# RoadlyInc/DSOPP

Hardware: AMD Instinct MI355X
Metric: Gauss-Newton iters/sec (7-KF window, 2k active pts) (higher is better)
Workload: dtype f64; 1 GPU; C1: 7-KF window, 2000 active points per GPU (2000 total, 2000 on rank 0), 640x480, full clique, production LM settings; frames=7, points_per_gpu=2000, total_points=2000, parallelism=single GPU, exchange=none, ranks=1

## Files before the change

dsopp_amd/csrc/pba_kernels.hpp:

```cpp
#pragma once
#include <type_traits>
#include "device_geom.hpp"
#include "pba_types.hpp"

namespace dsopp_hip {

__device__ __constant__ const int kPatX[kPat] = {0, -1, 1, -2, 0, 2, -1, 0};
__device__ __constant__ const int kPatY[kPat] = {2, 1, 1, 0, 0, 0, -1, -2};

__host__ __device__ constexpr int triIdx(int i, int j) { return i * kBlk - i * (i - 1) / 2 + (j - i); }
__host__ __device__ inline int symIdx(int i, int j) { return i <= j ? triIdx(i, j) : triIdx(j, i); }

__device__ inline void buildProjectionMatrices(const Rigid &T, const FrameDev &fr, const FrameDev &ft, double *U, double *M) {
  const double ifx = 1.0 / fr.fx, ify = 1.0 / fr.fy;
  const double k02 = -fr.cx / fr.fx, k12 = -fr.cy / fr.fy;
#pragma unroll
  for (int i = 0; i < 3; ++i) {
    U[4 * i + 0] = T.R[3 * i + 0] * ifx;
    U[4 * i + 1] = T.R[3 * i + 1] * ify;
    U[4 * i + 2] = T.R[3 * i + 0] * k02 + T.R[3 * i + 1] * k12 + T.R[3 * i + 2];
    U[4 * i + 3] = T.t[i];
  }
  if (M) {
#pragma unroll
    for (int j = 0; j < 4; ++j) {
      M[0 + j] = ft.fx * U[0 + j] + ft.cx * U[8 + j];
      M[4 + j] = ft.fy * U[4 + j] + ft.cy * U[8 + j];
      M[8 + j] = U[8 + j];
    }
  }
}

template <typename FramesPtr, typename StatePtr>
__device__ __forceinline__ double linearisationScale(FramesPtr frames, StatePtr st, int r, int t) {
  return (frames[t].exposure / frames[r].exposure) * exp(st->ab0[t][0] - st->ab0[r][0]);
}

template <typename StatePtr>
__device__ __forceinline__ Rigid frameIncrement(StatePtr st, int f, double sign) {
  double xi[6];
#pragma unroll
  for (int i = 0; i < 6; ++i) xi[i] = sign * (st->eps[f][i] + st->step[f][i]);
  return rigidExp(xi);
}

template <int PART = 0>
__device__ __forceinline__ void computePairConst(const FrameDev *frames_generic, const WindowState *st_generic, PairConst *pc_generic, int r, int t,
                                                 int F, bool fej, const Rigid *Er = nullptr, const Rigid *Emt = nullptr) {
  const auto frames = glb(frames_generic);
  const auto st = glb(st_generic);
  auto &P = glb(pc_generic)[r * kMaxFrames + t];
  const auto &fr = frames[r];
  const auto &ft = frames[t];
  const bool valid = (r != t) && fr.status[t] != nullptr;
  if (PART != 2) P.valid = valid ? 1 : 0;
  if (!valid) return;
  Rigid Tr0, Tt0;
#pragma unroll
  for (int i = 0; i < 9; ++i) {
    Tr0.R[i] = st->T0_R[r][i];
    Tt0.R[i] = st->T0_R[t][i];
  }
#pragma unroll
  for (int i = 0; i < 3; ++i) {
    Tr0.t[i] = st->T0_t[r][i];
    Tt0.t[i] = st->T0_t[t][i];
  }
  const Rigid T_tr0 = rigidMul(rigidInverse(Tt0), Tr0);
  if (PART != 1) {
#pragma unroll
    for (int i = 0; i < 3; ++i) {
#pragma unroll
      for (int j = 0; j < 3; ++j) P.T0rel[4 * i + j] = T_tr0.R[3 * i + j];
      P.T0rel[4 * i + 3] = T_tr0.t[i];
    }
  }
  FrameDev ir{}, it{};
  ir.fx = fr.fx;
  ir.fy = fr.fy;
  ir.cx = fr.cx;
  ir.cy = fr.cy;
  it.fx = ft.fx;
  it.fy = ft.fy;
  it.cx = ft.cx;
  it.cy = ft.cy;
  const bool need_current = PART != 2 || !fej;
  Rigid T_tr = T_tr0;
  double b_r = 0, s_cur = 0;
  if (need_current) {
    T_tr = rigidMul(Emt ? *Emt : frameIncrement(st, t, -1.0), rigidMul(T_tr0, Er ? *Er : frameIncrement(st, r, 1.0)));
    const double a_r = st->ab0[r][0] + st->eps[r][6] + st->step[r][6];
    const double a_t = st->ab0[t][0] + st->eps[t][6] + st->step[t][6];
    b_r = st->ab0[r][1] + st->eps[r][7] + st->step[r][7];
    s_cur = (ft.exposure / fr.exposure) * exp(a_t - a_r);
  }
  if (PART != 2) {
    const double b_t = st->ab0[t][1] + st->eps[t][7] + st->step[t][7];
    P.s = s_cur;
    P.b_t = b_t;
    P.b_r = b_r;
    double Ucur[12], Mcur[12];
    buildProjectionMatrices(T_tr, ir, it, Ucur, Mcur);
#pragma unroll
    for (int i = 0; i < 12; ++i) P.M[i] = Mcur[i];
  }
  if (PART != 1) {
    const Rigid Tlin = fej ? T_tr0 : T_tr;
    double Ulin[12], adj[36];
    buildProjectionMatrices(Tlin, ir, it, Ulin, nullptr);
    rigidAdj(Tlin, adj);
#pragma unroll
    for (int i = 0; i < 12; ++i) P.U[i] = Ulin[i];
#pragma unroll
    for (int i = 0; i < 36; ++i) P.Adj[i] = adj[i];
#pragma unroll
    for (int i = 0; i < 3; ++i) P.tl[i] = Tlin.t[i];
    P.fxt = ft.fx;
    P.fyt = ft.fy;
    P.cxt = ft.cx;
    P.cyt = ft.cy;
    if (fej) {
      P.s0 = linearisationScale(frames, st, r, t);
      P.b_r0 = st->ab0[r][1];
      int last = -1;
      for (int k = 0; k < F; ++k)
        if (k != r && fr.status[k] != nullptr) last = k;
      P.sigma_r = linearisationScale(frames, st, r, last);
    } else {
      P.s0 = s_cur;
      P.b_r0 = b_r;
      P.sigma_r = s_cur;
    }
  }
}

__device__ inline void refreshPairCurrent(const FrameDev *frames, const WindowState *st, PairConst *pc, int r, int t, const Rigid &Er,
                                          const Rigid &Emt) {
  PairConst &P = pc[r * kMaxFrames + t];
  if (!P.valid) return;
  Rigid T0;
#pragma unroll
  for (int i = 0; i < 3; ++i) {
#pragma unroll
    for (int j = 0; j < 3; ++j) T0.R[3 * i + j] = P.T0rel[4 * i + j];
    T0.t[i] = P.T0rel[4 * i + 3];
  }
  const Rigid T_tr = rigidMul(Emt, rigidMul(T0, Er));
  const FrameDev &fr = frames[r];
  const FrameDev &ft = frames[t];
  double U[12];
  buildProjectionMatrices(T_tr, fr, ft, U, P.M);
  const double a_r = st->ab0[r][0] + st->eps[r][6] + st->step[r][6];
  const double a_t = st->ab0[t][0] + st->eps[t][6] + st->step[t][6];
  P.s = (ft.exposure / fr.exposure) * exp(a_t - a_r);
  P.b_t = st->ab0[t][1] + st->eps[t][7] + st->step[t][7];
  P.b_r = st->ab0[r][1] + st->eps[r][7] + st->step[r][7];
}

__global__ void __launch_bounds__(kMaxFrames *kMaxFrames) pairSetupKernel(const FrameDev *frames, const WindowState *st, PairConst *pc, int F, int fej,
                                                                          const int *run_flag) {
  if (run_flag && !*run_flag) return;
  const int idx = threadIdx.x;
  if (idx >= F * F) return;
  computePairConst(frames, st, pc, idx / F, idx % F, F, fej != 0);
}

__device__ __forceinline__ double waveSum(double v) {
#pragma unroll
  for (int off = 32; off >= 1; off >>= 1) v += __shfl_xor(v, off, 64);
  return v;
}

__device__ __forceinline__ double waveSumDpp(double v) {
  auto mov = [](double x, auto ctrl_tag) {
    constexpr int CTRL = decltype(ctrl_tag)::value;
    int lo = __double2loint(x), hi = __double2hiint(x);
    lo = __builtin_amdgcn_mov_dpp(lo, CTRL, 0xF, 0xF, true);
    hi = __builtin_amdgcn_mov_dpp(hi, CTRL, 0xF, 0xF, true);
    return __hiloint2double(hi, lo);
  };
  v += mov(v, std::integral_constant<int, 0xB1>{});
  v += mov(v, std::integral_constant<int, 0x4E>{});
  v += mov(v, std::integral_constant<int, 0x141>{});
  v += mov(v, std::integral_constant<int, 0x140>{});
  auto row = [&](int lane) {
    const int lo = __builtin_amdgcn_readlane(__double2loint(v), lane), hi = __builtin_amdgcn_readlane(__double2hiint(v), lane);
    return __hiloint2double(hi, lo);
  };
  return ((row(0) + row(16)) + row(32)) + row(48);
}

template <int N, int THREADS>
__device__ __forceinline__ void blockSum(double (&vals)[N], double *lds ) {
  constexpr int kWaves = THREADS / 64;
  const int lane = threadIdx.x & 63, wave = threadIdx.x >> 6;
#pragma unroll
  for (int i = 0; i < N; ++i) vals[i] = waveSum(vals[i]);
  if (kWaves > 1) {
    if (lane == 0) {
#pragma unroll
      for (int i = 0; i < N; ++i) lds[wave * N + i] = vals[i];
    }
    __syncthreads();
    if (threadIdx.x == 0) {
#pragma unroll
      for (int i = 0; i < N; ++i) {
        double s = lds[i];
        for (int w = 1; w < kWaves; ++w) s += lds[w * N + i];
        vals[i] = s;
      }
    }
  }
}

constexpr int kItemsPerBlock = kSweepThreads / kPat;

template <typename S>
__global__ void __launch_bounds__(64) fejKernel(const FrameDev *__restrict__ frames, const PairConst *__restrict__ pc,
                                                const SweepBlock *__restrict__ table, int n_entries) {
  const int entry = blockIdx.x * (64 / kItemsPerBlock) + (threadIdx.x / kItemsPerBlock);
  if (entry >= n_entries) return;
  const SweepBlock be = table[entry];
  const FrameDev &fr = frames[be.r];
  const FrameDev &ft = frames[be.t];
  const PairConst &P = pc[be.r * kMaxFrames + be.t];
  const int i = be.offset + threadIdx.x % kItemsPerBlock;
  if (i >= fr.n_res[be.t]) return;
  const uint8_t flg = fr.flags[i];
  if ((flg & kFlagMarginalized) && !(flg & kFlagToMarginalize)) return;
  const S u = static_cast<S>(fr.uv[2 * i]), v = static_cast<S>(fr.uv[2 * i + 1]);
  const double idepth_d = fr.idepth[i];
  const S idepth = static_cast<S>(idepth_d);
  bool ok = validIdepth(idepth) && insideROI(u - S(2), v - S(2), S(fr.width), S(fr.height)) &&
            insideROI(u + S(2), v + S(2), S(fr.width), S(fr.height));
  const S U0 = S(P.U[0]), U1 = S(P.U[1]), U4 = S(P.U[4]), U5 = S(P.U[5]), U8 = S(P.U[8]), U9 = S(P.U[9]);
  const S cX = S(P.U[2]) + S(P.U[3]) * idepth, cY = S(P.U[6]) + S(P.U[7]) * idepth, cZ = S(P.U[10]) + S(P.U[11]) * idepth;
#pragma unroll
  for (int k = 0; k < kPat; ++k) {
    const S pu = u + S(kPatX[k]), pv = v + S(kPatY[k]);
    const S X = U0 * pu + U1 * pv + cX, Y = U4 * pu + U5 * pv + cY, Z = U8 * pu + U9 * pv + cZ;
    const S tu = (S(P.fxt) * X + S(P.cxt) * Z) / Z, tv = (S(P.fyt) * Y + S(P.cyt) * Z) / Z;
    ok = ok && (Z > S(0)) && insideROI(tu, tv, S(ft.width), S(ft.height));
  }
  fr.fej_valid[be.t][i] = ok ? 1 : 0;
  fr.idepth_fej[i] = idepth_d;
}

struct SweepParams {
  double sigma_huber;
  int for_marginalized;
  int use_fej_flag;
  const LmControl *ctrl;
  double *clear_buf;
  int clear_count;
  const double *step;
  double lambda;
  int F;
  int ublk_read, ublk_write;
  int gate_on_pending;
  const int *run_flag;
  int external_backsub;
  long long *dbg;
};
#ifdef DSOPP_HIP_STAMPS
constexpr bool kStamps = true;
#else
constexpr bool kStamps = false;
#endif
#define SWEEP_STAMP(i) do { if (kStamps && prm.dbg && threadIdx.x == 0 && blockIdx.x == gridDim.x / 2) prm.dbg[i] = wall_clock64(); } while (0)


__device__ __forceinline__ void ldsBarrier() { asm volatile("s_waitcnt lgkmcnt(0)\n\ts_barrier" ::: "memory"); }


template <int CTRL>
__device__ __forceinline__ double dppMove(double v) {
  int lo = __double2loint(v), hi = __double2hiint(v);
  lo = __builtin_amdgcn_mov_dpp(lo, CTRL, 0xF, 0xF, true);
  hi = __builtin_amdgcn_mov_dpp(hi, CTRL, 0xF, 0xF, true);
  return __hiloint2double(hi, lo);
}

__device__ __forceinline__ double sum8(double v) {
  v += dppMove<0xB1>(v);
  v += dppMove<0x4E>(v);
  v += dppMove<0x141>(v);
  return v;
}

__device__ __forceinline__ double fastRcp(double x) {
  double r = __builtin_amdgcn_rcp(x);
  r = fma(fma(-x, r, 1.0), r, r);
  r = fma(fma(-x, r, 1.0), r, r);
  return r;
}
__device__ __forceinline__ float fastRcp(float x) { return 1.0f / x; }

__device__ __forceinline__ double fastRsqrt(double x) {
  double y = __builtin_amdgcn_rsq(x);
  const double h = 0.5 * x;
  y = fma(y, fma(-h * y, y, 0.5), y);
  y = fma(y, fma(-h * y, y, 0.5), y);
  return y;
}

using f64x4 = __attribute__((ext_vector_type(4))) double;

constexpr int kGramStride = 18;
constexpr int kSweepScalars = 5;

__device__ __forceinline__ void gramPublish(const double (&a)[kBlk], const double (&b)[kBlk], double *wave_rows ) {
  const int lane = threadIdx.x & 63;
  double2 *row = reinterpret_cast<double2 *>(wave_rows + lane * kGramStride);
#pragma unroll
  for (int c = 0; c < kBlk / 2; ++c) {
    row[c] = double2{a[2 * c], a[2 * c + 1]};
    row[kBlk / 2 + c] = double2{b[2 * c], b[2 * c + 1]};
  }
}

__device__ __forceinline__ void gramContract(const double *wave_rows , f64x4 &acc) {
  const int lane = threadIdx.x & 63;
  __builtin_amdgcn_fence(__ATOMIC_RELEASE, "wavefront");
  __builtin_amdgcn_wave_barrier();
  __builtin_amdgcn_fence(__ATOMIC_ACQUIRE, "wavefront");
  const double *src = wave_rows + (4 * ((lane & 15) >> 3) + (lane >> 4)) * kGramStride + (lane & 7);
  double av[8], bv[8];
#pragma unroll
  for (int s = 0; s < 8; ++s) {
    av[s] = src[8 * s * kGramStride];
    bv[s] = src[8 * s * kGramStride + kBlk];
  }
  asm volatile("" ::: "memory");
#pragma unroll
  for (int s = 0; s < 8; ++s) acc = __builtin_amdgcn_mfma_f64_16x16x4f64(av[s], bv[s], acc, 0, 0, 0);
  __builtin_amdgcn_fence(__ATOMIC_RELEASE, "wavefront");
  __builtin_amdgcn_wave_barrier();
}

template <bool LIN>
__device__ __forceinline__ void gramScalarsStore(const f64x4 &acc, const double (&sc)[kSweepScalars], double *lds ,
                                                 double *__restrict__ out) {
  constexpr int kWaves = kSweepThreads / 64, kSlot = 64 + kSweepScalars;
  const int lane = threadIdx.x & 63, wave = threadIdx.x >> 6;
  const double e0 = acc[0] + dppMove<0x128>(acc[2]), e1 = acc[1] + dppMove<0x128>(acc[3]);
  double s[kSweepScalars];
#pragma unroll
  for (int i = 0; i < kSweepScalars; ++i) s[i] = waveSumDpp(sc[i]);
  const int col = lane & 15, r4 = lane >> 4;
  if (LIN && col < 8) {
    lds[wave * kSlot + 8 * r4 + col] = e0;
    lds[wave * kSlot + 8 * (r4 + 4) + col] = e1;
  }
  if (lane < kSweepScalars) {
    double v = s[0];
#pragma unroll
    for (int i = 1; i < kSweepScalars; ++i) v = lane == i ? s[i] : v;
    lds[wave * kSlot + 64 + lane] = v;
  }
  ldsBarrier();
  if (threadIdx.x < kSlot && (LIN || threadIdx.x >= 64)) {
    const int e = threadIdx.x;
    double v = lds[e];
#pragma unroll
    for (int w = 1; w < kWaves; ++w) v += lds[w * kSlot + e];
    int idx = -1;
    if (e < 64) {
      const int i = e >> 3, j = e & 7;
      if (i < 7) idx = j >= i ? triIdx(i, j) : -1;
      else idx = 36 + j;
    } else {
      idx = e - 64 < 4 ? 44 + (e - 64) : (LIN ? triIdx(7, 7) : -1);
    }
    if (idx >= 0) out[idx] = v;
  }
}

template <typename S, bool LIN, bool FEJ, bool HUBER, bool BACKSUB = false, bool WFEJ = false>
__global__ void __launch_bounds__(kSweepThreads) sweepKernel(const FrameDev *__restrict__ frames, const PairConst *__restrict__ pc,
                                                             const SweepBlock *__restrict__ table, double *__restrict__ partials,
                                                             const LmControl *ctrl_arg, const int *run_flag_arg,
                                                             SweepParams prm) {
  __shared__ __attribute__((aligned(16))) double gram_lds[LIN ? kSweepThreads * kGramStride : 2];
  __shared__ double scalar_lds[(kSweepThreads / 64) * (64 + kSweepScalars)];
  const SweepBlock be = table[blockIdx.x];
  static_assert(sizeof(SweepBlock) >= sizeof(LmControl) && sizeof(SweepBlock) >= sizeof(int), "the sweep table stands in for an absent control block / run flag");
  const LmControl DSOPP_CONSTANT *ctrl_or_any =
      ctrl_arg ? (const LmControl DSOPP_CONSTANT *)ctrl_arg : (const LmControl DSOPP_CONSTANT *)(const void DSOPP_CONSTANT *)table;
  const int DSOPP_CONSTANT *flag_or_any = run_flag_arg ? (const int DSOPP_CONSTANT *)run_flag_arg : (const int DSOPP_CONSTANT *)(const void DSOPP_CONSTANT *)table;
  int c_active = ctrl_or_any->active, c_lsv = ctrl_or_any->linear_system_valid, c_pending = ctrl_or_any->pending, run = *flag_or_any;
  double lam = ctrl_or_any->lambda;
  asm volatile("" ::"s"(be.r), "s"(be.t), "s"(be.offset), "s"(be.n_res), "s"(be.cap), "s"(be.owns_landmark_sums), "s"(be.width_r), "s"(be.height_r),
               "s"(be.width_t), "s"(be.height_t), "s"(be.conn_mask), "s"(be.n_groups), "s"(be.uv), "s"(be.idepth), "s"(be.patch), "s"(be.idepth_fej),
               "s"(be.b_d), "s"(be.inv_hdd), "s"(be.idepth_step), "s"(be.ublk), "s"(be.energy), "s"(be.flags), "s"(be.status), "s"(be.fej_valid),
               "s"(be.cand), "s"(be.texels_t), "s"(be.iplane_t), "s"(be.itiles_t), "s"(be.partial_row));
  asm volatile("" : "+s"(c_active), "+s"(c_lsv), "+s"(c_pending), "+s"(run), "+s"(lam));
  asm volatile("" ::"s"(prm.sigma_huber), "s"(prm.for_marginalized), "s"(prm.use_fej_flag), "s"(prm.clear_buf), "s"(prm.clear_count), "s"(prm.step),
               "s"(prm.lambda), "s"(prm.F), "s"(prm.ublk_read), "s"(prm.ublk_write), "s"(prm.gate_on_pending), "s"(prm.external_backsub), "s"(prm.dbg));
  if (!ctrl_arg) {
    c_active = 1;
    c_lsv = 0;
    c_pending = 1;
    lam = prm.lambda;
  }
  if (!run_flag_arg) run = 1;
  if (!run || !c_active || (LIN && c_lsv)) return;
  if (LIN && prm.clear_buf) {
    for (int k = blockIdx.x * kSweepThreads + threadIdx.x; k < prm.clear_count; k += gridDim.x * kSweepThreads) prm.clear_buf[k] = 0;
  }
  SWEEP_STAMP(0);
  const auto g_flags = glb(be.flags), g_status = glb(be.status), g_fej_valid = glb(be.fej_valid);
  const auto g_cand = glb(be.cand);
  const auto g_uv = glb(be.uv), g_idepth = glb(be.idepth), g_patch = glb(be.patch), g_idepth_fej = glb(be.idepth_fej);
  const auto g_b_d = glb(be.b_d), g_inv_hdd = glb(be.inv_hdd);
  const auto g_idepth_step = glb(be.idepth_step), g_ublk = glb(be.ublk), g_energy = glb(be.energy);
  const auto g_step = glb(prm.step);
  const PairConst DSOPP_CONSTANT &P = *(const PairConst DSOPP_CONSTANT *)(pc + (be.r * kMaxFrames + be.t));
  const int k = threadIdx.x & 7;
  const int ox = static_cast<int>((0x21420312u >> (4 * k)) & 0xFu) - 2;
  const int oy = static_cast<int>((0x01222334u >> (4 * k)) & 0xFu) - 2;

  double sc[kSweepScalars];
#pragma unroll
  for (int e = 0; e < kSweepScalars; ++e) sc[e] = 0;
  f64x4 gram = {0, 0, 0, 0};

  struct ItemWords {
    uint8_t flg, status, cand, fej_bit;
    S u, v, patch_k;
    double idepth_d, idepth_step_d, idepth_fej_d;
  };
  auto loadItemWords = [&](int item, bool in_bounds) {
    const int j = in_bounds ? item : be.offset;
    ItemWords w;
    w.flg = g_flags[j];
    w.u = static_cast<S>(g_uv[2 * j]);
    w.v = static_cast<S>(g_uv[2 * j + 1]);
    w.idepth_d = g_idepth[j];
    w.idepth_step_d = g_idepth_step[j];
    w.status = g_status[j];
    w.cand = g_cand[j];
    w.patch_k = static_cast<S>(g_patch[kPat * j + k]);
    w.fej_bit = 1;
    w.idepth_fej_d = 0;
    if (FEJ) {
      constexpr bool fresh_fej = LIN && WFEJ;
      if (prm.use_fej_flag && !fresh_fej) w.fej_bit = g_fej_valid[j];
      if (LIN) w.idepth_fej_d = fresh_fej ? w.idepth_d : g_idepth_fej[j];
    }
    return w;
  };
  ItemWords nxt;
  {
    const int i0 = be.offset + (threadIdx.x >> 3);
    nxt = loadItemWords(i0, i0 < be.n_res);
  }
  for (int grp = 0; grp < be.n_groups; ++grp) {
  const int i = be.offset + grp * kItemsPerBlock + (threadIdx.x >> 3);
  const PairConst DSOPP_CONSTANT *Pm = &P;
  asm volatile("" : "+s"(Pm) : "v"(i));

  const bool inb = i < be.n_res;
  uint8_t flg = 0;
  S u = S(0), v = S(0);
  double idepth_d = 0, idepth_step_d = 0, idepth_fej_d = 0, bd_d = 0, inv_hdd_d = 0;
  uint8_t status = DSOPP_HIP_STATUS_OOB, cand = DSOPP_HIP_STATUS_OOB;
  uint8_t fej_bit = 1;
  S patch_k = S(0);
  double hrow[kBlk], srow[kBlk];
#pragma unroll
  for (int c = 0; c < kBlk; ++c) hrow[c] = srow[c] = 0;
  const size_t plane = ublkPlane(be.cap);
  {
    const ItemWords cur = nxt;
    flg = cur.flg;
    u = cur.u;
    v = cur.v;
    idepth_d = cur.idepth_d;
    idepth_step_d = cur.idepth_step_d;
    status = cur.status;
    cand = cur.cand;
    patch_k = cur.patch_k;
    fej_bit = cur.fej_bit;
    idepth_fej_d = cur.idepth_fej_d;
  }
  if (inb) {
    if (BACKSUB) {
      bd_d = g_b_d[i];
      inv_hdd_d = g_inv_hdd[i];
      if (k < prm.F && (k == be.r || ((be.conn_mask >> k) & 1u))) {
        const auto src = g_ublk + (static_cast<size_t>(prm.ublk_read) * kMaxFrames + k) * plane + static_cast<size_t>(i) * kUblk;
#pragma unroll
        for (int c = 0; c < kBlk; ++c) {
          hrow[c] = src[c];
          srow[c] = g_step[kBlk * k + c];
        }
      }
    }
  }
  bool active = inb && !((flg & kFlagMarginalized) && !(flg & kFlagToMarginalize));
  const bool accumulate = active && (prm.for_marginalized ? (flg & kFlagToMarginalize) != 0 : (flg & kFlagMarginalized) == 0);
  bool fej_ok = fej_bit != 0;
  if (!active) {
    status = DSOPP_HIP_STATUS_OOB;
    cand = DSOPP_HIP_STATUS_OOB;
  }
  if (BACKSUB) {
    double d = 0;
    const bool upd = active && !(flg & (kFlagMarginalized | kFlagIllConditioned)) && (!prm.gate_on_pending || c_pending);
#pragma unroll
    for (int c = 0; c < kBlk; ++c) d += hrow[c] * srow[c];
    if (upd) {
      for (int tt = k + kPat; tt < prm.F; tt += kPat) {
        if (tt != be.r && !((be.conn_mask >> tt) & 1u)) continue;
        const auto src = g_ublk + (static_cast<size_t>(prm.ublk_read) * kMaxFrames + tt) * plane + static_cast<size_t>(i) * kUblk;
#pragma unroll
        for (int c = 0; c < kBlk; ++c) d += src[c] * g_step[kBlk * tt + c];
      }
    }
    d = sum8(d);
    if (upd) {
      idepth_step_d = -((bd_d - d) * (1.0 / (1.0 + lam)) * inv_hdd_d);
      if (k == 0 && be.owns_landmark_sums) g_idepth_step[i] = idepth_step_d;
    }
  }
  SWEEP_STAMP(1);
  if (kStamps && prm.dbg) asm volatile("s_waitcnt vmcnt(0)" ::: "memory");
  SWEEP_STAMP(2);
  const S idepth = static_cast<S>(idepth_d + idepth_step_d);
  const S Wr = S(be.width_r), Hr = S(be.height_r), Wt = S(be.width_t), Ht = S(be.height_t);

  const S pu = u + S(ox), pv = v + S(oy);
  S tu, tv;
  bool ok = active && validIdepth(idepth) && insideROI(pu, pv, Wr, Hr);
  if (!LIN || FEJ) {
    const S x = S(Pm->M[0]) * pu + S(Pm->M[1]) * pv + (S(Pm->M[2]) + S(Pm->M[3]) * idepth);
    const S y = S(Pm->M[4]) * pu + S(Pm->M[5]) * pv + (S(Pm->M[6]) + S(Pm->M[7]) * idepth);
    const S z = S(Pm->M[8]) * pu + S(Pm->M[9]) * pv + (S(Pm->M[10]) + S(Pm->M[11]) * idepth);
    const S iz = fastRcp(z);
    tu = x * iz;
    tv = y * iz;
    ok = ok && (z > S(0));
  } else {
    const S X = S(Pm->U[0]) * pu + S(Pm->U[1]) * pv + (S(Pm->U[2]) + S(Pm->U[3]) * idepth);
    const S Y = S(Pm->U[4]) * pu + S(Pm->U[5]) * pv + (S(Pm->U[6]) + S(Pm->U[7]) * idepth);
    const S Z = S(Pm->U[8]) * pu + S(Pm->U[9]) * pv + (S(Pm->U[10]) + S(Pm->U[11]) * idepth);
    tu = (S(Pm->fxt) * X + S(Pm->cxt) * Z) / Z;
    tv = (S(Pm->fyt) * Y + S(Pm->cyt) * Z) / Z;
    ok = ok && (Z > S(0));
  }
  ok = ok && insideROI(tu, tv, Wt, Ht);

  if (grp + 1 < be.n_groups) {
    const int in = i + kItemsPerBlock;
    nxt = loadItemWords(in, in < be.n_res);
    asm volatile("" ::: "memory");
  }
  S sI = S(0), sIx = S(0), sIy = S(0);
  double *const gram_rows = gram_lds + (LIN ? (threadIdx.x >> 6) * 64 * kGramStride : 0);
  if (!LIN && be.iplane_t != nullptr) {
    if (ok) {
      const int ix = static_cast<int>(tu), iy = static_cast<int>(tv);
      const S dx = tu - static_cast<S>(ix), dy = tv - static_cast<S>(iy);
      const S dxdy = dx * dy;
      const S w11 = dxdy, w01 = dy - dxdy, w10 = dx - dxdy, w00 = S(1) - dx - dy + dxdy;
      const int rx = static_cast<int>(floor(tu + S(0.5))) - ix, ry = static_cast<int>(floor(tv + S(0.5))) - iy;
      const int tiles = be.itiles_t;
      if constexpr (std::is_same<S, double>::value) {
        const auto ip = (GlobalPtr<const unsigned long long>)be.iplane_t;
        auto at = [&](int x, int y) { return ip[(static_cast<size_t>(y >> 1) * tiles + (x >> 2)) * 8 + ((y & 1) << 2) + (x & 3)]; };
        const unsigned long long b00 = at(ix, iy), b10 = at(ix + 1, iy), b01 = at(ix, iy + 1), b11 = at(ix + 1, iy + 1);
        const unsigned long long bm = ry ? (rx ? b11 : b01) : (rx ? b10 : b00);
        ok = (bm & 1ull) != 0;
        auto val = [](unsigned long long b) { return __longlong_as_double(static_cast<long long>(b & ~1ull)); };
        sI = w11 * val(b11) + w01 * val(b01) + w10 * val(b10) + w00 * val(b00);
      } else {
        const auto ip = (GlobalPtr<const unsigned>)be.iplane_t;
        auto at = [&](int x, int y) { return ip[(static_cast<size_t>(y >> 2) * tiles + (x >> 2)) * 16 + ((y & 3) << 2) + (x & 3)]; };
        const unsigned b00 = at(ix, iy), b10 = at(ix + 1, iy), b01 = at(ix, iy + 1), b11 = at(ix + 1, iy + 1);
        const unsigned bm = ry ? (rx ? b11 : b01) : (rx ? b10 : b00);
        ok = (bm & 1u) != 0;
        auto val = [](unsigned b) { return __uint_as_float(b & ~1u); };
        sI = w11 * val(b11) + w01 * val(b01) + w10 * val(b10) + w00 * val(b00);
      }
    }
  } else {
    Texel<S> t00{}, t10{}, t01{}, t11{};
    const int ix = static_cast<int>(tu), iy = static_cast<int>(tv);
    if (ok) {
      const Texel<S> *__restrict__ img = static_cast<const Texel<S> *>(be.texels_t);
      const int W = be.width_t;
      const Texel<S> *p = img + static_cast<size_t>(iy) * W + ix;
      t00 = loadTexel(p);
      t10 = loadTexel(p + 1);
      t01 = loadTexel(p + W);
      t11 = loadTexel(p + W + 1);
    }
    if (LIN && grp > 0) {
      __builtin_amdgcn_sched_barrier(0);
      gramContract(gram_rows, gram);
      __builtin_amdgcn_sched_barrier(0);
    }
    if (ok) {
      const S dx = tu - static_cast<S>(ix), dy = tv - static_cast<S>(iy);
      const S dxdy = dx * dy;
      const S w11 = dxdy, w01 = dy - dxdy, w10 = dx - dxdy, w00 = S(1) - dx - dy + dxdy;
      const int rx = static_cast<int>(floor(tu + S(0.5))) - ix, ry = static_cast<int>(floor(tv + S(0.5))) - iy;
      const S m = ry ? (rx ? t11.mask : t01.mask) : (rx ? t10.mask : t00.mask);
      ok = (m != S(0));
      sI = w11 * t11.I + w01 * t01.I + w10 * t10.I + w00 * t00.I;
      if (LIN) {
        sIx = w11 * t11.Ix + w01 * t01.Ix + w10 * t10.Ix + w00 * t00.Ix;
        sIy = w11 * t11.Iy + w01 * t01.Iy + w10 * t10.Iy + w00 * t00.Iy;
      }
    }
  }
  SWEEP_STAMP(3);
  const PairConst DSOPP_CONSTANT *Pj = &P;
  asm volatile("" : "+s"(Pj) : "v"(tu));
  const int shift = (threadIdx.x & 63) & ~7;
  if (FEJ && LIN && WFEJ) {
    const S idf = static_cast<S>(idepth_d);
    const S X = S(Pj->U[0]) * pu + S(Pj->U[1]) * pv + (S(Pj->U[2]) + S(Pj->U[3]) * idf);
    const S Y = S(Pj->U[4]) * pu + S(Pj->U[5]) * pv + (S(Pj->U[6]) + S(Pj->U[7]) * idf);
    const S Z = S(Pj->U[8]) * pu + S(Pj->U[9]) * pv + (S(Pj->U[10]) + S(Pj->U[11]) * idf);
    const S tuf = (S(Pj->fxt) * X + S(Pj->cxt) * Z) / Z, tvf = (S(Pj->fyt) * Y + S(Pj->cyt) * Z) / Z;
    const bool okf = (Z > S(0)) && insideROI(tuf, tvf, Wt, Ht);
    const unsigned long long fmask = __ballot(okf);
    const bool item_ok = (((fmask >> shift) & 0xFFull) == 0xFFull) && validIdepth(idf) && insideROI(u - S(2), v - S(2), Wr, Hr) &&
                         insideROI(u + S(2), v + S(2), Wr, Hr);
    if (prm.use_fej_flag) fej_ok = item_ok;
    if (active && k == 0) {
      glb(const_cast<uint8_t *>(static_cast<const uint8_t *>(be.fej_valid)))[i] = item_ok ? 1 : 0;
      glb(const_cast<double *>(static_cast<const double *>(be.idepth_fej)))[i] = idepth_d;
    }
  }
  const unsigned long long okmask = __ballot(ok);
  const bool success = active && fej_ok && (((okmask >> shift) & 0xFFull) == 0xFFull);

  if (active && !success) cand = DSOPP_HIP_STATUS_OOB;
  const bool evaluate = success && status == DSOPP_HIP_STATUS_OK;
  if (evaluate) cand = DSOPP_HIP_STATUS_OK;

  const S res = evaluate ? (sI - S(Pj->b_t)) - S(Pj->s) * (patch_k - S(Pj->b_r)) : S(0);
  const double r2 = sum8(static_cast<double>(res * res));
  double wgt = 1.0, energy = 0.5 * r2;
  if (HUBER) {
    const double sig = prm.sigma_huber;
    if (r2 > sig * sig) {
      const double inv_nrm = fastRsqrt(r2);
      const double nrm = r2 * inv_nrm;
      wgt = sig * inv_nrm;
      energy = sig * nrm - 0.5 * sig * sig;
    }
  }
  if (!evaluate) energy = 0;
  SWEEP_STAMP(10);

  if (LIN) {
    double gj[kBlk + 2];
    double ga[kBlk], gb[kBlk];
#pragma unroll
    for (int a = 0; a < kBlk + 2; ++a) gj[a] = 0;
#pragma unroll
    for (int a = 0; a < kBlk; ++a) ga[a] = gb[a] = 0;
    if (evaluate) {
      const S idj = FEJ ? static_cast<S>(idepth_fej_d) : idepth;
      const S X = S(Pj->U[0]) * pu + S(Pj->U[1]) * pv + (S(Pj->U[2]) + S(Pj->U[3]) * idj);
      const S Y = S(Pj->U[4]) * pu + S(Pj->U[5]) * pv + (S(Pj->U[6]) + S(Pj->U[7]) * idj);
      const S Z = S(Pj->U[8]) * pu + S(Pj->U[9]) * pv + (S(Pj->U[10]) + S(Pj->U[11]) * idj);
      const S fxt = S(Pj->fxt), fyt = S(Pj->fyt);
      const S rho = fastRcp(Z);
      const S b0 = X * rho, b1 = Y * rho;
      const S du_id = fxt * (S(Pj->tl[0]) * rho - S(Pj->tl[2]) * (rho * b0));
      const S dv_id = fyt * (S(Pj->tl[1]) * rho - S(Pj->tl[2]) * (rho * b1));
      const S nid = idj * rho;
      const S Iu = sIx, Iv = sIy;
      S g[kBlk];
      const S b0b1 = b0 * b1;
      g[0] = Iu * (fxt * nid);
      g[1] = Iv * (fyt * nid);
      g[2] = Iv * (fyt * (-nid * b1)) + Iu * (fxt * (-nid * b0));
      g[3] = Iv * (fyt * (-(b1 * b1 + S(1)))) + Iu * (fxt * (-b0b1));
      g[4] = Iv * (fyt * b0b1) + Iu * (fxt * (b0 * b0 + S(1)));
      g[5] = Iv * (fyt * b0) + Iu * (fxt * (-b1));
      g[6] = S(Pj->sigma_r) * (patch_k - S(Pj->b_r0));
      g[7] = S(1);
      const double jdd = static_cast<double>(Iu * du_id + Iv * dv_id);
      const double rk = static_cast<double>(res);
#pragma unroll
      for (int a = 0; a < kBlk; ++a) {
        const double wga = wgt * static_cast<double>(g[a]);
        gj[a] = wga * jdd;
        if (a < kBlk - 1) {
          ga[a] = accumulate ? wga : 0.0;
          gb[a] = static_cast<double>(g[a]);
        }
      }
      ga[kBlk - 1] = accumulate ? wgt * rk : 0.0;
      gb[kBlk - 1] = 1.0;
      if (accumulate) sc[4] += wgt;
      gj[8] = wgt * jdd * jdd;
      gj[9] = wgt * jdd * rk;
    }
    SWEEP_STAMP(11);
    gramPublish(ga, gb, gram_rows);
    SWEEP_STAMP(12);
    {
      const bool b0 = (k & 1) != 0, b1 = (k & 2) != 0, b2 = (k & 4) != 0;
      double ra[4];
#pragma unroll
      for (int j = 0; j < 4; ++j) {
        const double keep = b2 ? gj[2 * j + 1] : gj[2 * j], send = b2 ? gj[2 * j] : gj[2 * j + 1];
        ra[j] = keep + dppMove<0x141>(send);
      }
      double rb[2];
#pragma unroll
      for (int m = 0; m < 2; ++m) {
        const double keep = b0 ? ra[2 * m + 1] : ra[2 * m], send = b0 ? ra[2 * m] : ra[2 * m + 1];
        rb[m] = keep + dppMove<0xB1>(send);
      }
      const double u_tot = (b1 ? rb[1] : rb[0]) + dppMove<0x4E>(b1 ? rb[0] : rb[1]);
      double hb = (b2 ? gj[9] : gj[8]) + dppMove<0x141>(b2 ? gj[8] : gj[9]);
      hb += dppMove<0xB1>(hb);
      hb += dppMove<0x4E>(hb);
      if (active) {
        const auto dst = g_ublk + (static_cast<size_t>(prm.ublk_write) * kMaxFrames + be.t) * plane + static_cast<size_t>(i) * kUblk;
        dst[((k & 3) << 1) | (k >> 2)] = -u_tot;
        if ((k & 3) == 0) dst[8 + (k >> 2)] = hb;
      }
    }
  }
  SWEEP_STAMP(13);
  if (active && k == 0) {
    g_energy[i] = energy;
    g_cand[i] = cand;
    if (accumulate) {
      sc[0] += energy;
      sc[1] += energy > 0 ? 1.0 : 0.0;
    }
    if ((!LIN || BACKSUB || prm.external_backsub) && be.owns_landmark_sums) {
      sc[2] += (prm.gate_on_pending && !c_pending) ? idepth_d * idepth_d : idepth_step_d * idepth_step_d;
      sc[3] += idepth_d * idepth_step_d;
    }
  }
  }
  SWEEP_STAMP(14);
  if (LIN && be.n_groups > 0) gramContract(gram_lds + (threadIdx.x >> 6) * 64 * kGramStride, gram);
  SWEEP_STAMP(4);
  double *out = partials + static_cast<size_t>(be.partial_row) * kPartial;
  gramScalarsStore<LIN>(gram, sc, scalar_lds, out);
  SWEEP_STAMP(5);
  SWEEP_STAMP(6);
  if (kStamps && prm.dbg && threadIdx.x == 0) {
    atomicMin(reinterpret_cast<unsigned long long *>(prm.dbg + 8), static_cast<unsigned long long>(wall_clock64()));
    atomicMax(reinterpret_cast<unsigned long long *>(prm.dbg + 9), static_cast<unsigned long long>(wall_clock64()));
  }
}

}
```

Before: 27620 GN iterations/s.

## Batch wave reductions, prefetch constant pair data, and restructure sweep loop tail

Five unrelated micro-optimizations land together. The per-scalar DPP wave sums are merged into one interleaved routine that issues all five reductions per stage for more ILP and reuses the local row-0 value instead of a readlane. Scalar loads of PairConst fields are touched early to prefetch constant data, with an explicit s_waitcnt inserted. The group loop becomes a do-while with an early exit that zeroes partials for empty blocks, which removes the n_groups check before the final gram contraction. A TAIL variant pins the MFMA operand registers. The early exit must zero exactly the slots the normal path writes, and the hand-coded waitcnt value is fragile.

Measured after the change: 27920 GN iterations/s, median of 6. 1.1% higher.

```diff
diff --git a/dsopp_amd/csrc/pba_kernels.hpp b/dsopp_amd/csrc/pba_kernels.hpp
--- a/dsopp_amd/csrc/pba_kernels.hpp
+++ b/dsopp_amd/csrc/pba_kernels.hpp
@@ -171,23 +171,38 @@
   return v;
 }
 
-__device__ __forceinline__ double waveSumDpp(double v) {
-  auto mov = [](double x, auto ctrl_tag) {
+template <int N>
+__device__ __forceinline__ void waveSumsDppRow0(const double (&v)[N], double (&total)[N]) {
+  double t[N], m[N];
+#pragma unroll
+  for (int i = 0; i < N; ++i) t[i] = v[i];
+  auto stage = [&](auto ctrl_tag) {
     constexpr int CTRL = decltype(ctrl_tag)::value;
-    int lo = __double2loint(x), hi = __double2hiint(x);
-    lo = __builtin_amdgcn_mov_dpp(lo, CTRL, 0xF, 0xF, true);
-    hi = __builtin_amdgcn_mov_dpp(hi, CTRL, 0xF, 0xF, true);
-    return __hiloint2double(hi, lo);
+#pragma unroll
+    for (int i = 0; i < N; ++i) {
+      int lo = __double2loint(t[i]), hi = __double2hiint(t[i]);
+      lo = __builtin_amdgcn_mov_dpp(lo, CTRL, 0xF, 0xF, true);
+      hi = __builtin_amdgcn_mov_dpp(hi, CTRL, 0xF, 0xF, true);
+      m[i] = __hiloint2double(hi, lo);
+    }
+#pragma unroll
+    for (int i = 0; i < N; ++i) t[i] += m[i];
   };
-  v += mov(v, std::integral_constant<int, 0xB1>{});
-  v += mov(v, std::integral_constant<int, 0x4E>{});
-  v += mov(v, std::integral_constant<int, 0x141>{});
-  v += mov(v, std::integral_constant<int, 0x140>{});
-  auto row = [&](int lane) {
-    const int lo = __builtin_amdgcn_readlane(__double2loint(v), lane), hi = __builtin_amdgcn_readlane(__double2hiint(v), lane);
-    return __hiloint2double(hi, lo);
-  };
-  return ((row(0) + row(16)) + row(32)) + row(48);
+  stage(std::integral_constant<int, 0xB1>{});
+  stage(std::integral_constant<int, 0x4E>{});
+  stage(std::integral_constant<int, 0x141>{});
+  stage(std::integral_constant<int, 0x140>{});
+  double r[3][N];
+#pragma unroll
+  for (int k = 0; k < 3; ++k) {
+#pragma unroll
+    for (int i = 0; i < N; ++i) {
+      const int lo = __builtin_amdgcn_readlane(__double2loint(t[i]), 16 * (k + 1)), hi = __builtin_amdgcn_readlane(__double2hiint(t[i]), 16 * (k + 1));
+      r[k][i] = __hiloint2double(hi, lo);
+    }
+  }
+#pragma unroll
+  for (int i = 0; i < N; ++i) total[i] = ((t[i] + r[0][i]) + r[1][i]) + r[2][i];
 }
 
 template <int N, int THREADS>
@@ -319,6 +334,7 @@
   }
 }
 
+template <bool TAIL = false>
 __device__ __forceinline__ void gramContract(const double *wave_rows , f64x4 &acc) {
   const int lane = threadIdx.x & 63;
   __builtin_amdgcn_fence(__ATOMIC_RELEASE, "wavefront");
@@ -331,6 +347,10 @@
     av[s] = src[8 * s * kGramStride];
     bv[s] = src[8 * s * kGramStride + kBlk];
   }
+  if (TAIL) {
+    asm volatile("" : "+v"(av[0]), "+v"(av[1]), "+v"(av[2]), "+v"(av[3]), "+v"(av[4]), "+v"(av[5]), "+v"(av[6]), "+v"(av[7]), "+v"(bv[0]), "+v"(bv[1]),
+                 "+v"(bv[2]), "+v"(bv[3]), "+v"(bv[4]), "+v"(bv[5]), "+v"(bv[6]), "+v"(bv[7]));
+  }
   asm volatile("" ::: "memory");
 #pragma unroll
   for (int s = 0; s < 8; ++s) acc = __builtin_amdgcn_mfma_f64_16x16x4f64(av[s], bv[s], acc, 0, 0, 0);
@@ -345,8 +365,7 @@
   const int lane = threadIdx.x & 63, wave = threadIdx.x >> 6;
   const double e0 = acc[0] + dppMove<0x128>(acc[2]), e1 = acc[1] + dppMove<0x128>(acc[3]);
   double s[kSweepScalars];
-#pragma unroll
-  for (int i = 0; i < kSweepScalars; ++i) s[i] = waveSumDpp(sc[i]);
+  waveSumsDppRow0(sc, s);
   const int col = lane & 15, r4 = lane >> 4;
   if (LIN && col < 8) {
     lds[wave * kSlot + 8 * r4 + col] = e0;
@@ -450,15 +469,27 @@
     }
     return w;
   };
+  if (be.n_groups <= 0) {
+    double *row = partials + static_cast<size_t>(be.partial_row) * kPartial;
+    if (threadIdx.x < kPartial && (LIN || threadIdx.x >= 44)) row[threadIdx.x] = 0;
+    return;
+  }
   ItemWords nxt;
   {
     const int i0 = be.offset + (threadIdx.x >> 3);
     nxt = loadItemWords(i0, i0 < be.n_res);
   }
-  for (int grp = 0; grp < be.n_groups; ++grp) {
+  int grp = 0;
+  do {
   const int i = be.offset + grp * kItemsPerBlock + (threadIdx.x >> 3);
   const PairConst DSOPP_CONSTANT *Pm = &P;
   asm volatile("" : "+s"(Pm) : "v"(i));
+  constexpr bool kTouch = std::is_same<S, double>::value;
+  if (kTouch && (!LIN || FEJ)) {
+    const int DSOPP_CONSTANT *w = (const int DSOPP_CONSTANT *)(const void DSOPP_CONSTANT *)&P;
+    asm volatile("" : "+s"(w) : "v"(i));
+    asm volatile("" ::"s"(w[offsetof(PairConst, M) / 4]), "s"(w[offsetof(PairConst, M) / 4 + 16]), "s"(w[offsetof(PairConst, U) / 4 - 1]));
+  }
 
   const bool inb = i < be.n_res;
   uint8_t flg = 0;
@@ -601,6 +632,12 @@
       gramContract(gram_rows, gram);
       __builtin_amdgcn_sched_barrier(0);
     }
+    if (kTouch) {
+      const int DSOPP_CONSTANT *w = (const int DSOPP_CONSTANT *)(const void DSOPP_CONSTANT *)&P;
+      asm volatile("" : "+s"(w) : "v"(tu));
+      if (LIN) asm volatile("" ::"s"(w[offsetof(PairConst, U) / 4]), "s"(w[offsetof(PairConst, U) / 4 + 16]), "s"(w[offsetof(PairConst, Adj) / 4 - 1]));
+      asm volatile("" ::"s"(w[offsetof(PairConst, fxt) / 4]), "s"(w[offsetof(PairConst, fxt) / 4 + 16]), "s"(w[offsetof(PairConst, b_r0) / 4 + 1]));
+    }
     if (ok) {
       const S dx = tu - static_cast<S>(ix), dy = tv - static_cast<S>(iy);
       const S dxdy = dx * dy;
@@ -615,6 +652,7 @@
       }
     }
   }
+  __builtin_amdgcn_s_waitcnt(0x0F70);
   SWEEP_STAMP(3);
   const PairConst DSOPP_CONSTANT *Pj = &P;
   asm volatile("" : "+s"(Pj) : "v"(tu));
@@ -744,9 +782,9 @@
       sc[3] += idepth_d * idepth_step_d;
     }
   }
-  }
+  } while (++grp < be.n_groups);
   SWEEP_STAMP(14);
-  if (LIN && be.n_groups > 0) gramContract(gram_lds + (threadIdx.x >> 6) * 64 * kGramStride, gram);
+  if (LIN) gramContract<true>(gram_lds + (threadIdx.x >> 6) * 64 * kGramStride, gram);
   SWEEP_STAMP(4);
   double *out = partials + static_cast<size_t>(be.partial_row) * kPartial;
   gramScalarsStore<LIN>(gram, sc, scalar_lds, out);
```
